# d0-rb/slim-switch-moe-vit

Measured on AMD Instinct MI355X. Metric: images/sec (fwd) ViT-B/16 E=8 @224^2, higher is better.
Workload: dtype f16; 1 GPU; ViT-B/16 Switch-MoE E=8 top-1, 224^2, batch 256/GPU, full eval forward (12 blocks: attention + MoE MLP), fp16 autocast; global_batch=256, compute_streams=1, parallelism=single

## Files before the change

slim-switch-moe-vit_amd/csrc/gemm.hip:

```cpp
#include "smoe_common.h"
#include <type_traits>
#include <cstdlib>

namespace {

typedef __bf16 bf16x8_t __attribute__((ext_vector_type(8)));

constexpr int BM = 128, BN = 128, BK_BYTES = 128;
constexpr int GEMM_THREADS = 256;
constexpr int STAGE_BYTES = (BM + BN) * BK_BYTES;
constexpr int C_PAD = 16;

__device__ __forceinline__ float gelu_erf(float v) {
  const float a = fabsf(v);
  const float z = a * 0.70710678118654752440f;
  const float t = __builtin_amdgcn_rcpf(fmaf(0.3275911f, z, 1.0f));
  float p = fmaf(t, 1.061405429f, -1.453152027f);
  p = fmaf(p, t, 1.421413741f);
  p = fmaf(p, t, -0.284496736f);
  p = fmaf(p, t, 0.254829592f);
  p *= t;
  const float ex = __builtin_amdgcn_exp2f(z * z * -1.4426950408889634f);
  const float erf_abs = fmaf(-p, ex, 1.0f);
  return 0.5f * fmaf(a, erf_abs, v);
// ... 1062 lines not shown
  hipLaunchKernelGGL(kern, dim3(grid), dim3(512), smem, s, (const AB*)PT, (const AB*)QT, (const float*)nullptr, offsets_pad,
                     (const int32_t*)nullptr, E, Lp, R2, (int)SMOE_EPI_NONE, (const int64_t*)nullptr, (const float*)nullptr,
                     (const float*)nullptr, out, tn, tm, R1, (const int64_t*)nullptr, 1);
  SMOE_CHECK_LAUNCH("smoe_grouped_wgrad");
  return 0;
}

template <typename AB>
int launch_wgrad_rows(const void* P, const void* Q, const int32_t* offsets, const int32_t* group_end, int E, int R1, int R2,
                      const void* zero16, float* out, hipStream_t s) {
  constexpr int TBN = 256;
  const int tn = (R2 + TBN - 1) / TBN, tm4 = (R1 + 255) / 256, tm5 = (R1 + 319) / 320;
  const int64_t cus = smoe_num_cus();
  const double c4 = (double)(((int64_t)E * tm4 * tn + cus - 1) / cus), c5 = 1.25 * (double)(((int64_t)E * tm5 * tn + cus - 1) / cus);
  if (c5 < c4) {
    const size_t smem = 2 * (size_t)(320 + TBN) * BK_BYTES;
    auto kern = grouped_gemm_pp256<AB, float, 0, 2, 5>;
    SMOE_ENSURE_SMEM(grouped_gemm_pp256<AB, float, 0, 2, 5>);
    hipLaunchKernelGGL(kern, dim3(E * tm5 * tn), dim3(512), smem, s, (const AB*)P, (const AB*)Q, (const float*)nullptr, offsets,
                       group_end, E, 0, R2, (int)SMOE_EPI_NONE, (const int64_t*)nullptr, (const float*)nullptr,
                       (const float*)zero16, out, tn, tm5, R1, (const int64_t*)nullptr, 1);
  } else {
    const size_t smem = 2 * (size_t)(256 + TBN) * BK_BYTES;
    auto kern = grouped_gemm_pp256<AB, float, 0, 2>;
    SMOE_ENSURE_SMEM(grouped_gemm_pp256<AB, float, 0, 2>);
    hipLaunchKernelGGL(kern, dim3(E * tm4 * tn), dim3(512), smem, s, (const AB*)P, (const AB*)Q, (const float*)nullptr, offsets,
                       group_end, E, 0, R2, (int)SMOE_EPI_NONE, (const int64_t*)nullptr, (const float*)nullptr,
                       (const float*)zero16, out, tn, tm4, R1, (const int64_t*)nullptr, 1);
  }
  SMOE_CHECK_LAUNCH("smoe_grouped_wgrad_rows");
  return 0;
}

template <typename AB, typename OT>
int launch_variant(int variant, const void* A, const void* W, const float* bias, const int32_t* offsets,
                   const int32_t* group_expert, int E, int64_t m_rows_max, int K, int N, int epilogue,
                   const int64_t* row_map, const float* row_scale, const void* residual, void* out, hipStream_t s,
                   const int64_t* a_gather, int a_div, const int32_t* group_end, int64_t out_rows) {
  if constexpr (sizeof(AB) == 2) {
    switch (variant) {
      case 1: return launch_glds<AB, OT, 128, 128, 2, 2, 2>(A, W, bias, offsets, group_expert, E, m_rows_max, K, N, epilogue, row_map, row_scale, residual, out, 8, s);
      case 2: return launch_glds<AB, OT, 256, 128, 2, 2, 1>(A, W, bias, offsets, group_expert, E, m_rows_max, K, N, epilogue, row_map, row_scale, residual, out, 4, s);
      case 3: return launch_glds<AB, OT, 256, 256, 2, 4, 2>(A, W, bias, offsets, group_expert, E, m_rows_max, K, N, epilogue, row_map, row_scale, residual, out, 4, s);
      case 4: {
        const int ntn = (N + 255) / 256;
        const int64_t t256 = ((m_rows_max + 255) / 256 + E / 2) * ntn, t320 = ((m_rows_max + 319) / 320 + E / 2) * ntn;
        const int cus = smoe_num_cus();
        const double c256 = (double)((t256 + cus - 1) / cus) * 1.0, c320 = (double)((t320 + cus - 1) / cus) * 1.25;
        const bool deep = K >= 2048;
        if (c320 <= c256) {
          if (deep) return launch_pp256<AB, OT, 16, 5>(A, W, bias, offsets, group_expert, E, m_rows_max, K, N, epilogue, row_map, row_scale, residual, out, 4, s, a_gather, a_div);
          return launch_pp256<AB, OT, 0, 5>(A, W, bias, offsets, group_expert, E, m_rows_max, K, N, epilogue, row_map, row_scale, residual, out, 4, s, a_gather, a_div);
        }
        if (deep) return launch_pp256<AB, OT, 16, 4>(A, W, bias, offsets, group_expert, E, m_rows_max, K, N, epilogue, row_map, row_scale, residual, out, 4, s, a_gather, a_div);
        return launch_pp256<AB, OT>(A, W, bias, offsets, group_expert, E, m_rows_max, K, N, epilogue, row_map, row_scale, residual, out, 4, s, a_gather, a_div);
      }
#ifdef SMOE_DIAG
      case 5: {
        const char* gm = getenv("SMOE_GROUP_M");
        return launch_pp256<AB, OT, 0, 5>(A, W, bias, offsets, group_expert, E, m_rows_max, K, N, epilogue, row_map, row_scale, residual, out, gm ? atoi(gm) : 4, s, a_gather, a_div);
      }
#else
      case 5: return launch_pp256<AB, OT, 0, 5>(A, W, bias, offsets, group_expert, E, m_rows_max, K, N, epilogue, row_map, row_scale, residual, out, 4, s, a_gather, a_div);
#endif
      case 9: {
        const int ntn = (N + 255) / 256;
        const int64_t t256 = ((m_rows_max + 255) / 256 + E / 2) * ntn, t320 = ((m_rows_max + 319) / 320 + E / 2) * ntn;
        const int cus = smoe_num_cus();
        const double c256 = (double)((t256 + cus - 1) / cus) * 1.0, c320 = (double)((t320 + cus - 1) / cus) * 1.25;
        const bool deep = K >= 2048;
        if (c320 <= c256) {
          if (deep) return launch_ps<AB, OT, 5, true>(A, W, bias, offsets, group_expert, E, m_rows_max, K, N, epilogue, row_map, row_scale, residual, out, 4, s, a_gather, a_div, group_end, out_rows);
          return launch_ps<AB, OT, 5, false>(A, W, bias, offsets, group_expert, E, m_rows_max, K, N, epilogue, row_map, row_scale, residual, out, 4, s, a_gather, a_div, group_end, out_rows);
        }
        if (deep) return launch_ps<AB, OT, 4, true>(A, W, bias, offsets, group_expert, E, m_rows_max, K, N, epilogue, row_map, row_scale, residual, out, 4, s, a_gather, a_div, group_end, out_rows);
        return launch_ps<AB, OT, 4, false>(A, W, bias, offsets, group_expert, E, m_rows_max, K, N, epilogue, row_map, row_scale, residual, out, 4, s, a_gather, a_div, group_end, out_rows);
      }
      case 14: {
        const int ntn = (N + 255) / 256;
        const int64_t t256 = ((m_rows_max + 255) / 256 + E / 2) * ntn, t320 = ((m_rows_max + 319) / 320 + E / 2) * ntn;
        const int cus = smoe_num_cus();
        const double c256 = (double)((t256 + cus - 1) / cus) * 1.0, c320 = (double)((t320 + cus - 1) / cus) * 1.25;
        const bool deep = K >= 2048;
        if (c320 <= c256) {
          if (deep) return launch_ps<AB, OT, 5, true>(A, W, bias, offsets, group_expert, E, m_rows_max, K, N, epilogue, row_map, row_scale, residual, out, 4, s, a_gather, a_div, group_end, out_rows, false);
          return launch_ps<AB, OT, 5, false>(A, W, bias, offsets, group_expert, E, m_rows_max, K, N, epilogue, row_map, row_scale, residual, out, 4, s, a_gather, a_div, group_end, out_rows, false);
        }
        if (deep) return launch_ps<AB, OT, 4, true>(A, W, bias, offsets, group_expert, E, m_rows_max, K, N, epilogue, row_map, row_scale, residual, out, 4, s, a_gather, a_div, group_end, out_rows, false);
        return launch_ps<AB, OT, 4, false>(A, W, bias, offsets, group_expert, E, m_rows_max, K, N, epilogue, row_map, row_scale, residual, out, 4, s, a_gather, a_div, group_end, out_rows, false);
      }
      case 10: return launch_ps<AB, OT, 5, false>(A, W, bias, offsets, group_expert, E, m_rows_max, K, N, epilogue, row_map, row_scale, residual, out, 4, s, a_gather, a_div, group_end, out_rows);
      case 11: return launch_ps<AB, OT, 4, false>(A, W, bias, offsets, group_expert, E, m_rows_max, K, N, epilogue, row_map, row_scale, residual, out, 4, s, a_gather, a_div, group_end, out_rows);
      case 12: return launch_ps<AB, OT, 4, true>(A, W, bias, offsets, group_expert, E, m_rows_max, K, N, epilogue, row_map, row_scale, residual, out, 4, s, a_gather, a_div, group_end, out_rows);
      case 13: return launch_ps<AB, OT, 5, true>(A, W, bias, offsets, group_expert, E, m_rows_max, K, N, epilogue, row_map, row_scale, residual, out, 4, s, a_gather, a_div, group_end, out_rows);
      case 6: return launch_pp256<AB, OT>(A, W, bias, offsets, group_expert, E, m_rows_max, K, N, epilogue, row_map, row_scale, residual, out, 4, s, a_gather, a_div);
      case 7: return launch_pp256<AB, OT, 16, 4>(A, W, bias, offsets, group_expert, E, m_rows_max, K, N, epilogue, row_map, row_scale, residual, out, 4, s, a_gather, a_div);
      case 8: return launch_pp256<AB, OT, 16, 5>(A, W, bias, offsets, group_expert, E, m_rows_max, K, N, epilogue, row_map, row_scale, residual, out, 4, s, a_gather, a_div);
#ifdef SMOE_DIAG
      case 41: return launch_pp256<AB, OT, 1>(A, W, bias, offsets, group_expert, E, m_rows_max, K, N, epilogue, row_map, row_scale, residual, out, 4, s);
      case 42: return launch_pp256<AB, OT, 2>(A, W, bias, offsets, group_expert, E, m_rows_max, K, N, epilogue, row_map, row_scale, residual, out, 4, s);
      case 43: return launch_pp256<AB, OT, 3>(A, W, bias, offsets, group_expert, E, m_rows_max, K, N, epilogue, row_map, row_scale, residual, out, 4, s);
      case 44: return launch_pp256<AB, OT, 4>(A, W, bias, offsets, group_expert, E, m_rows_max, K, N, epilogue, row_map, row_scale, residual, out, 4, s);
      case 46: return launch_pp256<AB, OT, 6>(A, W, bias, offsets, group_expert, E, m_rows_max, K, N, epilogue, row_map, row_scale, residual, out, 4, s);
      case 48: return launch_pp256<AB, OT, 8>(A, W, bias, offsets, group_expert, E, m_rows_max, K, N, epilogue, row_map, row_scale, residual, out, 4, s);
      case 47: return launch_pp256<AB, OT, 7>(A, W, bias, offsets, group_expert, E, m_rows_max, K, N, epilogue, row_map, row_scale, residual, out, 4, s);
#endif
      default: break;
    }
  }
  return launch_t128<AB, OT>(A, W, bias, offsets, group_expert, E, m_rows_max, K, N, epilogue, row_map, row_scale, residual, out, s);
}

template <typename AB>
int dispatch_out(int variant, const void* A, const void* W, const float* bias, const int32_t* offsets, const int32_t* group_expert,
                 int E, int64_t m_rows_max, int K, int N, int epilogue, const int64_t* row_map, const float* row_scale,
                 const void* residual, void* out, int out_dtype, hipStream_t s, const int64_t* a_gather, int a_div,
                 const int32_t* group_end, int64_t out_rows) {
  switch (out_dtype) {
    case SMOE_F32: return launch_variant<AB, float>(variant, A, W, bias, offsets, group_expert, E, m_rows_max, K, N, epilogue, row_map, row_scale, residual, out, s, a_gather, a_div, group_end, out_rows);
    case SMOE_F16: return launch_variant<AB, f16>(variant, A, W, bias, offsets, group_expert, E, m_rows_max, K, N, epilogue, row_map, row_scale, residual, out, s, a_gather, a_div, group_end, out_rows);
    case SMOE_BF16: return launch_variant<AB, bf16_bits>(variant, A, W, bias, offsets, group_expert, E, m_rows_max, K, N, epilogue, row_map, row_scale, residual, out, s, a_gather, a_div, group_end, out_rows);
  }
  smoe_set_error("smoe_grouped_gemm: bad out_dtype %d", out_dtype);
// ... 20 lines not shown
  const size_t cap = sizeof(unsigned long long) * 1024 * 8;
  return (int)hipMemcpyFromSymbol(host_out, HIP_SYMBOL(smoe_clock_stamps), n * 8 < cap ? n * 8 : cap);
}
extern "C" int smoe_clock_clear_stamps() {
  static unsigned long long z[1024 * 8];
  return (int)hipMemcpyToSymbol(HIP_SYMBOL(smoe_clock_stamps), z, sizeof(z));
}
#endif

extern "C" int smoe_grouped_gemm(const void* A, const void* W, const float* bias, const int32_t* offsets,
                                 const int32_t* group_expert, int G, int n_experts, int64_t m_rows_max, int K, int N,
                                 int ab_dtype, int epilogue, const int64_t* row_map, const float* row_scale,
                                 const void* residual, const int64_t* a_gather, int a_div, void* out, int64_t out_rows,
                                 int out_dtype, int variant, const int32_t* group_end, void* stream) {
  SMOE_REQUIRE(offsets && G >= 1 && G <= 65536, "smoe_grouped_gemm: bad G=%d / offsets", G);
  SMOE_REQUIRE(n_experts >= 1 && (group_expert || n_experts == G), "smoe_grouped_gemm: n_experts=%d != G=%d without a group map", n_experts, G);
  SMOE_REQUIRE(m_rows_max >= 0 && m_rows_max < (1ll << 31), "smoe_grouped_gemm: m_rows_max=%lld out of range",
               (long long)m_rows_max);
  SMOE_REQUIRE(K > 0 && N > 0, "smoe_grouped_gemm: bad K=%d N=%d", K, N);
  SMOE_REQUIRE(out_rows >= 0 && (out_rows == 0 || row_map || out_rows >= m_rows_max),
               "smoe_grouped_gemm: out_rows=%lld is smaller than m_rows_max=%lld", (long long)out_rows, (long long)m_rows_max);
  if (out_rows == 0 && !row_map) out_rows = m_rows_max;
  SMOE_REQUIRE(epilogue == SMOE_EPI_NONE || epilogue == SMOE_EPI_GELU || epilogue == SMOE_EPI_GELU_GRAD,
               "smoe_grouped_gemm: bad epilogue %d", epilogue);
  SMOE_REQUIRE(epilogue != SMOE_EPI_GELU_GRAD || (residual && !row_map),
               "smoe_grouped_gemm: SMOE_EPI_GELU_GRAD needs the pre-activations in `residual` and no row_map");
  SMOE_REQUIRE(smoe_dtype_ok(ab_dtype) && smoe_dtype_ok(out_dtype), "smoe_grouped_gemm: bad dtype");
  const int bke = BK_BYTES / smoe_dtype_size(ab_dtype);
  SMOE_REQUIRE(K % bke == 0, "smoe_grouped_gemm: K=%d must be a multiple of %d for this dtype", K, bke);
  SMOE_REQUIRE(N % 8 == 0, "smoe_grouped_gemm: N=%d must be a multiple of 8", N);
  if (m_rows_max == 0) return 0;
  SMOE_REQUIRE(A && W && out, "smoe_grouped_gemm: null pointer");
  if (K % 64 != 0 || smoe_dtype_size(ab_dtype) != 2) variant = 0;
  SMOE_REQUIRE(!a_gather || (variant >= 4 && variant <= 14 && a_div >= 1),
               "smoe_grouped_gemm: a_gather needs variant 4-14 (16-bit operands, K %% 64 == 0)");
  if (variant >= 9 && variant <= 14) {
    const uint64_t a_bytes = (uint64_t)m_rows_max * (uint64_t)K * 2u, w_bytes = (uint64_t)n_experts * (uint64_t)N * (uint64_t)K * 2u;
    if (a_bytes >= (1ull << 32) || w_bytes >= (1ull << 32) || G > 63) variant = variant == 14 ? 4 : variant - 5;
  }
  SMOE_REQUIRE(!group_end || (variant >= 9 && variant <= 14),
               "smoe_grouped_gemm: group_end (separate row ranges per group) needs the persistent kernel: variant 9-14, 16-bit "
               "operands under 4 GiB, K %% 64 == 0, at most 63 groups");
  hipStream_t s = (hipStream_t)stream;
  switch (ab_dtype) {
    case SMOE_F32: return dispatch_out<float>(variant, A, W, bias, offsets, group_expert, G, m_rows_max, K, N, epilogue, row_map, row_scale, residual, out, out_dtype, s, a_gather, a_div, group_end, out_rows);
    case SMOE_F16: return dispatch_out<f16>(variant, A, W, bias, offsets, group_expert, G, m_rows_max, K, N, epilogue, row_map, row_scale, residual, out, out_dtype, s, a_gather, a_div, group_end, out_rows);
    case SMOE_BF16: return dispatch_out<bf16_bits>(variant, A, W, bias, offsets, group_expert, G, m_rows_max, K, N, epilogue, row_map, row_scale, residual, out, out_dtype, s, a_gather, a_div, group_end, out_rows);
  }
  return 1;
}

#ifdef SMOE_FFN_FUSED
extern "C" size_t smoe_expert_ffn_workspace_bytes(int64_t m_rows_max, int G) {
  return sizeof(int32_t) * (size_t)(FUSED_WS_HDR + (m_rows_max + 319) / 320 + (G > 0 ? G : 0) + 8);
}
extern "C" int smoe_expert_ffn(const void* X, const int64_t* a_gather, int a_div, const void* W1, const float* b1, void* H,
                               const void* W2, const float* b2, const int32_t* offsets, const int32_t* group_expert, int G,
                               int n_experts, int64_t m_rows_max, int d_in, int d_hidden, int d_out, int ab_dtype,
                               const int64_t* row_map, const float* row_scale, const void* residual, void* out, int64_t out_rows,
                               int out_dtype, void* workspace, size_t workspace_bytes, void* stream) {
  SMOE_REQUIRE(offsets && G >= 1 && n_experts >= 1 && (group_expert || n_experts == G), "smoe_expert_ffn: bad groups");
  SMOE_REQUIRE(m_rows_max >= 0 && m_rows_max < (1ll << 31) && d_in > 0 && d_hidden > 0 && d_out > 0, "smoe_expert_ffn: bad sizes");
  SMOE_REQUIRE(a_div >= 1, "smoe_expert_ffn: a_div must be >= 1");
  if (m_rows_max == 0) return 0;
  SMOE_REQUIRE(X && W1 && H && W2 && out && workspace, "smoe_expert_ffn: null pointer");
  SMOE_REQUIRE(workspace_bytes >= smoe_expert_ffn_workspace_bytes(m_rows_max, G), "smoe_expert_ffn: workspace too small");
  if ((ab_dtype != SMOE_F16 && ab_dtype != SMOE_BF16) || out_dtype != SMOE_F32) return -1;
  if (d_in % 64 || d_hidden % 64 || d_out % 8 || G > 63) return -1;
  const uint64_t x_bytes = (uint64_t)m_rows_max * (uint64_t)(d_in > d_hidden ? d_in : d_hidden) * 2u;
  const uint64_t w_bytes = (uint64_t)n_experts * (uint64_t)d_hidden * (uint64_t)(d_in > d_out ? d_in : d_out) * 2u;
  if (x_bytes >= (1ull << 32) || w_bytes >= (1ull << 32)) return -1;
  if (out_rows <= 0 || out_rows * (int64_t)d_out * 4 >= (1ll << 31)) return -1;
  if ((int64_t)d_hidden * 320 * 2 >= (1ll << 31)) return -1;
  const int ntn1 = (d_hidden + 255) / 256, ntn2 = (d_out + 255) / 256;
// ... 66 lines not shown
```

slim-switch-moe-vit_amd/csrc/gemm_persistent.h:

```cpp
#ifndef PS_STORE_AUX
#define PS_STORE_AUX 0
#endif
#ifdef SMOE_DIAG
__device__ unsigned long long smoe_diag_stamps[256 * 12 * 16];
__device__ int smoe_diag_flags;
#define PS_NODMA (diag_nodma)
#define PS_IBAR() do { if (!diag_nobar) PP_BARRIER(); } while (0)
#define PS_STAMP(i)                                                                                              \
  do {                                                                                                           \
    if (wave == 0 && lane == 0 && tile_no < 12 && blockIdx.x < 256)                                              \
      smoe_diag_stamps[(blockIdx.x * 12 + tile_no) * 16 + (i)] = __builtin_amdgcn_s_memtime();                   \
  } while (0)
#else
#define PS_STAMP(i) do {} while (0)
#define PS_NODMA false
#define PS_IBAR() PP_BARRIER()
#endif

#ifdef SMOE_CLOCK
__device__ unsigned long long smoe_clock_stamps[1024 * 8];
#define PS_CLOCK(i)                                                                                             \
  do {                                                                                                          \
    if (wave == 0 && lane == 0 && blockIdx.x < 1024) {                                                          \
      unsigned long long t_sh, t_rt;                                                                            \
// ... 14 lines not shown
constexpr int FUSED_WS_HDR = 32;
constexpr int FUSED_WS_LEFT = 16, FUSED_WS_ERR = 17;
constexpr int FUSED_SPIN_LIMIT = 1 << 22;
struct FusedCtl {
  int32_t* ws;
  int mt_lo, cnt;
  int n1, n2, A, B2, G;
  int ntn1, ntn2, gm;
  int stage, slot, j;
  int nk, nid;
};
__device__ __forceinline__ void fused_advance(FusedCtl& fc) {
  if (fc.stage == 1) {
    const int id = fc.slot + fc.G * fc.j;
    if (id < fc.A) { fc.nk = 1; fc.nid = id; ++fc.j; return; }
    fc.nk = 0;
    return;
  }
  if (fc.stage == 2) {
    if (fc.slot < fc.B2) {
      if (fc.j == 0) { fc.nk = 2; fc.nid = fc.slot; fc.j = 1; return; }
    } else {
      const int id = fc.A + (fc.slot - fc.B2) + (fc.G - fc.B2) * fc.j;
      if (id < fc.n1) { fc.nk = 1; fc.nid = id; ++fc.j; return; }
    }
    fc.stage = 3;
    fc.j = 0;
  }
  const int f = fc.B2 + fc.slot + fc.G * fc.j;
  if (f < fc.n2) { fc.nk = 2; fc.nid = f; ++fc.j; return; }
  fc.nk = 0;
}

template <typename AB, typename OT, int AFR, bool DEEP, bool KEEP, bool DIRECT, bool BUF, int FUSED>
__device__ __forceinline__ void ps_body(
    const AB* __restrict__ A, const AB* __restrict__ W, const float* __restrict__ bias,
    const int32_t* __restrict__ offsets, const int32_t* __restrict__ group_expert, int E, int K, int N, int epilogue,
    const int64_t* __restrict__ row_map, const float* __restrict__ row_scale, const OT* residual, OT* out, int n_tiles_n,
    int group_m, const int64_t* __restrict__ a_gather, int a_div, int gather_len, const int32_t* __restrict__ group_end,
    FusedCtl* fc) {
  static_assert(sizeof(AB) == 2, "16-bit operands");
  static_assert(FUSED == 0 || (!KEEP && ((FUSED == 1 && DIRECT) || (FUSED == 2 && BUF))), "fused roles: 1 = producer (direct 16-bit stores), 2 = consumer");
  static_assert(!DIRECT || (sizeof(OT) == 2 && !KEEP), "the direct epilogue stores 16-bit outputs, one output per tile");
  extern __shared__ __attribute__((aligned(16))) char smem[];
  constexpr int TBM = 64 * AFR, TBN = 256, NT = 512, NW = 8;
  constexpr int STAGE = (TBM + TBN) * BK_BYTES;
  constexpr int ASLOTS = TBM / 8 / NW;
  constexpr int SLOTS = 4;
  constexpr int LDS_TOTAL = 160 * 1024;

  const int tid = threadIdx.x, lane = tid & 63;
  const int wave = __builtin_amdgcn_readfirstlane(tid >> 6);
  const int wr = wave >> 2, wc = wave & 3;
  const int fr = lane & 15, fq = lane >> 4;
  const int nk = K / 64;
#ifdef SMOE_DIAG
  const bool diag_nodma = (__builtin_amdgcn_readfirstlane(smoe_diag_flags) & 1) != 0;
  const bool diag_nobar = (__builtin_amdgcn_readfirstlane(smoe_diag_flags) & 2) != 0;
#endif

  int t_off = 0, t_end = 0, t_tb = 0, t_ge = lane;
  {
    const int li = lane < E ? lane : (group_end ? E - 1 : E);
    t_off = offsets[li];
    t_end = group_end ? group_end[li] : offsets[li < E ? li + 1 : E];
    int cnt = lane < E ? (t_end - t_off + TBM - 1) / TBM : 0;
    int incl = cnt;
#pragma unroll
    for (int sft = 1; sft < 64; sft <<= 1) {
      const int up = __shfl_up(incl, sft, 64);
      if (lane >= sft) incl += up;
    }
    t_tb = incl - cnt;
    if (group_expert && lane < E) t_ge = group_expert[lane];
  }
  const int total_mt = __builtin_amdgcn_readlane(t_tb, 63);
// ... 240 lines not shown
    if (a_gather && wave < TBM / 64) {
      int gr = m0 + wave * 64 + lane;
      if (gr >= m_end) gr = m_end - 1;
      __builtin_amdgcn_global_load_lds((const __attribute__((address_space(1))) void*)(a_gather + gr),
                                       (__attribute__((address_space(3))) void*)(smem + LDS_TOTAL - 2048 - TBM * 4 + wave * 256),
                                       4, 0, 0);
    }
  };
  auto issue_bias = [&](int par) {
    if (bias && wave == 0) {
      int col = n0 + lane * 4;
      if (col > N - 4) col = N - 4;
      PS_DMA(bias + (int64_t)e * N + col, bias_lds + par * 1024);
    }
  };

  if constexpr (FUSED == 0) {
    if (!advance()) return;
  } else {
    locate_fused(fc->nid);
    if constexpr (FUSED == 2) fused_wait(mt_next, fused_poll(mt_next));
  }
  if constexpr (FUSED == 0) PS_CLOCK(0);
  {
    int oz = 0;
    asm volatile("" : "+v"(oz));
    setup(lane + oz);
  }
  issue_bias(0);
  issue_kt0();
  if (nk > 1) {
    issue_kt1();
    if constexpr (DEEP) wait_keep2();
    else if constexpr (AFR == 4) asm volatile("s_waitcnt vmcnt(8)" ::: "memory");
    else asm volatile("s_waitcnt vmcnt(9)" ::: "memory");
  } else {
    asm volatile("s_waitcnt vmcnt(0)" ::: "memory");
  }
  PP_BARRIER();

  int tile_no = 0;
  (void)tile_no;
  int cmt = 0;
  for (;; ++tile_no) {
    PS_STAMP(0);
    const int ce = e, cm0 = m0, cm_end = m_end, cn0 = n0;
    cmt = mt_next;
    if constexpr (FUSED != 0) PS_COUNT(4 + FUSED, 1);
    bool more;
    if constexpr (FUSED == 0) {
      tile += t_step;
      more = advance();
    } else {
      fused_advance(*fc);
      more = fc->nk == FUSED;
      if (more) {
        locate_fused(fc->nid);
        if constexpr (FUSED == 2) polled = fused_poll(mt_next);
      }
    }
    if (more) prefetch_rows();
#pragma unroll
    for (int i = 0; i < 2 * AFR; ++i)
#pragma unroll
      for (int j = 0; j < 4; ++j) acc[i][j] = f32x4{0.f, 0.f, 0.f, 0.f};
    if (wr == 1) PP_BARRIER();
    if constexpr (DEEP) {
      for (int t = 0; t < nk; ++t) {
        const int cur = t & 1, nxt = cur ^ 1;
        const bool n1 = (t + 1 < nk), n2 = (t + 2 < nk);
        read_b(cur, 0);
        __builtin_amdgcn_sched_barrier(0);
        read_a(cur, 0);
        if (n1) dma_ah(t + 1, nxt, 1);
        PS_IBAR();
        PS_MFMA(0, 0);
        PS_IBAR();
        read_b(cur, 1);
        if (n1) dma_wh(t + 1, nxt, 0);
        PS_IBAR();
        PS_MFMA(0, 1);
        PS_IBAR();
        read_a(cur, 1);
        if (n2) dma_ah(t + 2, cur, 0);
        PS_IBAR();
        PS_MFMA(1, 1);
        PS_IBAR();
        read_b(cur, 0);
        if (n2) dma_wh(t + 2, cur, 1);
        if (wr == 1) {
          if (n2) wait_keep2();
          else asm volatile("s_waitcnt vmcnt(0)" ::: "memory");
        }
        PS_IBAR();
        PS_MFMA(1, 0);
        if (wr == 0) {
          if (n2) wait_keep2();
          else asm volatile("s_waitcnt vmcnt(0)" ::: "memory");
        }
        PS_IBAR();
      }
    } else {
      for (int t = 0; t < nk; ++t) {
        const int cur = t & 1, nxt = cur ^ 1;
        const bool pre1 = (t >= 1) && (t + 1 < nk);
        const bool pre2 = (t + 2 < nk);
        read_b(cur, 0);
        __builtin_amdgcn_sched_barrier(0);
        read_a(cur, 0);
        if (pre1) dma_a(t + 1, nxt, 2);
        PS_IBAR();
        PS_MFMA(0, 0);
        PS_IBAR();
        read_b(cur, 1);
        if (pre1) dma_w(t + 1, nxt, 0);
        PS_IBAR();
        PS_MFMA(0, 1);
        PS_IBAR();
        read_a(cur, 1);
        if (pre1) dma_w(t + 1, nxt, 2);
        PS_IBAR();
        PS_MFMA(1, 1);
        PS_IBAR();
        read_b(cur, 0);
        if (pre2) dma_a(t + 2, cur, 0);
        if (wr == 1) {
          if (pre2) asm volatile("s_waitcnt vmcnt(2)" ::: "memory");
          else asm volatile("s_waitcnt vmcnt(0)" ::: "memory");
        }
        PS_IBAR();
        PS_MFMA(1, 0);
        if (wr == 0) {
          if (pre2) asm volatile("s_waitcnt vmcnt(2)" ::: "memory");
          else asm volatile("s_waitcnt vmcnt(0)" ::: "memory");
        }
        PS_IBAR();
      }
    }
    if (wr == 0) PP_BARRIER();
    PS_STAMP(1);
    if constexpr (FUSED != 0) {
      if (mt_done >= 0) fused_signal(mt_done);
    }

    PS_STAMP(2);
    int oz = 0;
    asm volatile("" : "+v"(oz));
    const int tid_e = tid + oz, lane_e = tid_e & 63;
    if (more) {
      if constexpr (FUSED == 2) fused_wait(mt_next, polled);
      rows_in_lds = a_gather != nullptr;
      setup(lane_e);
      issue_bias(bias_par ^ 1);
      PS_STAMP(3);
      issue_kt0();
      if constexpr (DIRECT && DEEP) issue_kt1();
    }
    PS_STAMP(4);

    if constexpr (DIRECT) {
      (void)ce;
      const int fr = lane_e & 15, fq = lane_e >> 4;
      f32x4 bv[4];
#pragma unroll
      for (int ni = 0; ni < 4; ++ni) {
        const int nl = wc * 64 + ni * 16 + fq * 4;
        bv[ni] = f32x4{0.f, 0.f, 0.f, 0.f};
        if (bias) bv[ni] = *reinterpret_cast<const f32x4*>(bias_lds + bias_par * 1024 + nl * 4);
      }
      bias_par ^= 1;
      const int rows_here = (cm_end - cm0 < TBM) ? (cm_end - cm0) : TBM;
      const __amdgpu_buffer_rsrc_t rs = __builtin_amdgcn_make_buffer_rsrc(
          reinterpret_cast<char*>(out) + (int64_t)cm0 * N * 2, 0, rows_here * N * 2, 0x00020000);
      const int cq = wc * 64 + (fq & 1) * 16 + (fq >> 1) * 8;
      const uint32_t OOR = 0x80000000u;
      uint32_t off0 = (uint32_t)(((wr * (TBM / 2) + fr) * N + cn0 + cq) * 2);
      const bool ok0 = cn0 + cq < N, ok1 = cn0 + cq + 32 < N;
      const uint32_t row16 = (uint32_t)(16 * N * 2);
#pragma unroll
      for (int mi = 0; mi < 2 * AFR; ++mi) {
#pragma unroll
        for (int q = 0; q < 2; ++q) {
          f32x4 va = acc[mi][2 * q] + bv[2 * q], vb = acc[mi][2 * q + 1] + bv[2 * q + 1];
          if (epilogue == SMOE_EPI_GELU) { va = gelu_fast4(va); vb = gelu_fast4(vb); }
          uint32_t a0, a1, b0, b1;
          pack4<OT>(va, a0, a1);
          pack4<OT>(vb, b0, b1);
          const auto s0 = __builtin_amdgcn_permlane16_swap(a0, b0, false, false);
          const auto s1 = __builtin_amdgcn_permlane16_swap(a1, b1, false, false);
          const u32x4 v = u32x4{s0[0], s1[0], s0[1], s1[1]};
          const uint32_t off = off0 + (uint32_t)(q * 64);
#ifdef FUSED_EXP_PLAIN_STORES
          __builtin_amdgcn_raw_buffer_store_b128(v, rs, (int)((q ? ok1 : ok0) ? off : OOR), 0, PS_STORE_AUX);
#else
          __builtin_amdgcn_raw_buffer_store_b128(v, rs, (int)((q ? ok1 : ok0) ? off : OOR), 0, FUSED == 1 ? 16 : PS_STORE_AUX);
#endif
        }
        off0 += row16;
      }
      PS_STAMP(5);
      if (!more) break;
      if constexpr (DEEP) {
        if constexpr (AFR == 5) asm volatile("s_waitcnt vmcnt(20)" ::: "memory");
        else asm volatile("s_waitcnt vmcnt(16)" ::: "memory");
      } else {
        issue_kt1();
        if (nk > 1) {
          if constexpr (AFR == 5) asm volatile("s_waitcnt vmcnt(29)" ::: "memory");
          else asm volatile("s_waitcnt vmcnt(24)" ::: "memory");
        } else {
          if constexpr (AFR == 5) asm volatile("s_waitcnt vmcnt(20)" ::: "memory");
          else asm volatile("s_waitcnt vmcnt(16)" ::: "memory");
        }
      }
      PP_BARRIER();
      PS_STAMP(12);
      if constexpr (FUSED == 1) mt_done = cmt;
      continue;
    }

    (void)ce;
    const int fr = lane_e & 15, fq = lane_e >> 4;
    const int trow = tid_e / TPR, tcol = tid_e % TPR;
    f32x4 bv[NI];
#pragma unroll
    for (int ni = 0; ni < NI; ++ni) {
      const int nl = wc * TN + ni * 16 + fq * 4;
      bv[ni] = f32x4{0.f, 0.f, 0.f, 0.f};
      if (bias) bv[ni] = *reinterpret_cast<const f32x4*>(bias_lds + bias_par * 1024 + nl * 4);
    }
    bias_par ^= 1;
    const bool use_omap = OMAP && row_map != nullptr;
    if (use_omap && tid_e < TBM) {
      const int m = cm0 + tid_e;
// ... 178 lines not shown
            if (ncol < N) *reinterpret_cast<u32x4*>(reinterpret_cast<char*>(out) + (rbase + ncol) * OB) = v[j];
          }
          if constexpr (KEEP) {
#pragma unroll
            for (int j = 0; j < CPT; ++j) {
              const int ncol = cn0 + (tcol + j * TPR) * (16 / OB);
              const u32x4 h2 = *reinterpret_cast<const u32x4*>(cst2 + r * C_STRIDE + (tcol + j * TPR) * 16);
              if (ncol < N) *reinterpret_cast<u32x4*>(reinterpret_cast<char*>(pre_out) + (rbase + ncol) * OB) = h2;
            }
          }
        }
#pragma unroll
        for (int j = 0; j < CPT; ++j) resv[j] = resn[j];
      }
      if (p == 0) PS_STAMP(7);
      if (p == NPASS - 1) PS_STAMP(11);
      asm volatile("s_waitcnt lgkmcnt(0)" ::: "memory");
      PP_BARRIER();
    }
    PS_STAMP(12);
    if (!more) break;
    issue_kt1();
  }
  if constexpr (FUSED == 0) PS_CLOCK(2);
  if constexpr (FUSED != 0) {
    asm volatile("s_waitcnt vmcnt(0) lgkmcnt(0)" ::: "memory");
    PP_BARRIER();
    if constexpr (FUSED == 1) fused_signal(cmt);
  }
#undef PS_MFMA
#undef PS_DMA
}

template <typename AB, typename OT, int AFR, bool DEEP, bool KEEP = false, bool DIRECT = false, bool BUF = false>
__global__ __launch_bounds__(512, 2) void grouped_gemm_ps(
    const AB* __restrict__ A, const AB* __restrict__ W, const float* __restrict__ bias,
    const int32_t* __restrict__ offsets, const int32_t* __restrict__ group_expert, int E, int K, int N, int epilogue,
    const int64_t* __restrict__ row_map, const float* __restrict__ row_scale, const OT* residual, OT* out, int n_tiles_n,
    int group_m, const int64_t* __restrict__ a_gather, int a_div, int gather_len, const int32_t* __restrict__ group_end) {
  ps_body<AB, OT, AFR, DEEP, KEEP, DIRECT, BUF, 0>(A, W, bias, offsets, group_expert, E, K, N, epilogue, row_map, row_scale, residual,
                                                   out, n_tiles_n, group_m, a_gather, a_div, gather_len, group_end, nullptr);
}

struct FusedPlan { int A, B2; };
__device__ __forceinline__ FusedPlan fused_plan(int cnt, int ntn1, int ntn2, int G, int gm, int c1, int c2) {
  FusedPlan p;
  const int n1 = cnt * ntn1, n2 = cnt * ntn2;
  const int q2 = n2 / G, rem2 = n2 % G;
  p.A = n1;
  p.B2 = 0;
  if (c1 > 0 && rem2 > 0 && rem2 < G) {
    int best_x = -1, best_cost = 0x7fffffff;
    const int x_hi = n1 / G;
    for (int x = x_hi; x >= 0 && x >= x_hi - 8; --x) {
      const int left = n1 - x * G;
      const int y = x + (left + (G - rem2) - 1) / (G - rem2);
      const int heavy = x * c1 + (q2 + 1) * c2, light = y * c1 + q2 * c2;
      const int cost = heavy > light ? heavy : light;
      if (cost < best_cost) { best_cost = cost; best_x = x; }
    }
    const int A = best_x * G;
    const int early_cap = (A / (gm * ntn1)) * gm * ntn2;
    const int B2 = rem2 < early_cap ? rem2 : early_cap;
    if (A < n1 && B2 > 0) { p.A = A; p.B2 = B2; }
  }
  return p;
}

#ifdef SMOE_FFN_FUSED
template <typename AB>
__global__ __launch_bounds__(512, 2) void expert_ffn_fused(
    const AB* __restrict__ X, const int64_t* __restrict__ a_gather, int a_div, int gather_len, const AB* __restrict__ W1,
    const float* __restrict__ b1, AB* H, const AB* __restrict__ W2, const float* __restrict__ b2,
// ... 58 lines not shown
      }
    }
  };
  while (t1 < fc.G) {
    fc.stage = 1;
    fc.slot = t1;
    run_slot();
    if (tid == 0) slot2[0] = __hip_atomic_fetch_add(ws + home, 1, __ATOMIC_RELAXED, __HIP_MEMORY_SCOPE_AGENT);
    __syncthreads();
    t1 = __builtin_amdgcn_readfirstlane(slot2[0]);
    __syncthreads();
  }
  if (t2 < fc.G) {
    const int L = fc.G - fc.B2;
    fc.stage = 2;
    fc.slot = t2 < L ? fc.B2 + t2 : t2 - L;
    run_slot();
  }
  PS_CLOCK(2);
  __syncthreads();
  if (tid == 0) {
    asm volatile("s_waitcnt vmcnt(0)" ::: "memory");
    slot2[0] = __hip_atomic_fetch_add(ws + FUSED_WS_LEFT, 1, __ATOMIC_RELAXED, __HIP_MEMORY_SCOPE_AGENT);
  }
  __syncthreads();
  if (slot2[0] == (int)gridDim.x - 1) {
    for (int i = tid; i < FUSED_WS_HDR + total_mt; i += 512)
      if (i != FUSED_WS_ERR) __hip_atomic_store(ws + i, 0, __ATOMIC_RELAXED, __HIP_MEMORY_SCOPE_AGENT);
  }
}

#endif

template <typename AB, typename OT, int AFR, bool DEEP, bool KEEP = false>
int launch_ps(const void* A, const void* W, const float* bias, const int32_t* offsets, const int32_t* group_expert, int E,
              int64_t m_rows_max, int K, int N, int epilogue, const int64_t* row_map, const float* row_scale,
              const void* residual, void* out, int group_m, hipStream_t s, const int64_t* a_gather, int a_div,
              const int32_t* group_end, int64_t out_rows, bool allow_direct = true) {
  constexpr int TBM = 64 * AFR, TBN = 256;
  const int n_tiles_n = (N + TBN - 1) / TBN;
  const int64_t max_tiles = ((m_rows_max + TBM - 1) / TBM + E) * n_tiles_n;
  int grid = (smoe_num_cus() - smoe_reserved_cus()) & ~7;
  if (grid < 8) grid = 8;
  if (max_tiles < grid) grid = (int)((max_tiles + 7) & ~(int64_t)7);
  int n_block = n_tiles_n <= 4 ? n_tiles_n : 0;
#ifdef SMOE_DIAG
  if (const char* gcap = getenv("SMOE_PS_GRID")) grid = atoi(gcap) & ~7;
  if (const char* ord = getenv("SMOE_PS_NBLOCK")) n_block = atoi(ord);
  if (n_block && n_tiles_n % n_block) n_block = 0;
#endif
  if (n_block) group_m = -(group_m | (n_block << 8));
  if constexpr (!KEEP && sizeof(OT) == 2) {
    if (allow_direct && !row_map && !residual && (epilogue == SMOE_EPI_NONE || epilogue == SMOE_EPI_GELU) && (int64_t)N * TBM * 2 < (1ll << 31)) {
      SMOE_ENSURE_SMEM(grouped_gemm_ps<AB, OT, AFR, DEEP, false, true>);
      hipLaunchKernelGGL((grouped_gemm_ps<AB, OT, AFR, DEEP, false, true>), dim3(grid), dim3(512), 160 * 1024, s, (const AB*)A,
                         (const AB*)W, bias, offsets, group_expert, E, K, N, epilogue, row_map, row_scale, (const OT*)residual,
                         (OT*)out, n_tiles_n, group_m, a_gather, a_div, (int)m_rows_max, group_end);
      SMOE_CHECK_LAUNCH("smoe_grouped_gemm/persistent-direct");
      return 0;
    }
  }
  if constexpr (!KEEP && sizeof(OT) == 4) {
    if (allow_direct && epilogue != SMOE_EPI_GELU_GRAD && out_rows > 0 && out_rows * (int64_t)N * 4 < (1ll << 31)) {
      SMOE_ENSURE_SMEM(grouped_gemm_ps<AB, OT, AFR, DEEP, false, false, true>);
      hipLaunchKernelGGL((grouped_gemm_ps<AB, OT, AFR, DEEP, false, false, true>), dim3(grid), dim3(512), 160 * 1024, s,
                         (const AB*)A, (const AB*)W, bias, offsets, group_expert, E, K, N, epilogue, row_map, row_scale,
                         (const OT*)residual, (OT*)out, n_tiles_n, group_m, a_gather, a_div, (int)m_rows_max, group_end);
      SMOE_CHECK_LAUNCH("smoe_grouped_gemm/persistent-buffer");
      return 0;
    }
  }
  SMOE_ENSURE_SMEM(grouped_gemm_ps<AB, OT, AFR, DEEP, KEEP>);
  hipLaunchKernelGGL((grouped_gemm_ps<AB, OT, AFR, DEEP, KEEP>), dim3(grid), dim3(512), 160 * 1024, s, (const AB*)A, (const AB*)W,
                     bias, offsets, group_expert, E, K, N, epilogue, row_map, row_scale, (const OT*)residual, (OT*)out,
                     n_tiles_n, group_m, a_gather, a_div, (int)m_rows_max, group_end);
  SMOE_CHECK_LAUNCH("smoe_grouped_gemm/persistent");
  return 0;
}
```

Measured before the change: 21610 images/s.

## Add skewed tile-boundary schedule to persistent direct-epilogue grouped GEMM

```diff
diff --git a/slim-switch-moe-vit_amd/csrc/gemm.hip b/slim-switch-moe-vit_amd/csrc/gemm.hip
--- a/slim-switch-moe-vit_amd/csrc/gemm.hip
+++ b/slim-switch-moe-vit_amd/csrc/gemm.hip
@@ -1118,6 +1118,24 @@
   return 0;
 }
 
+template <typename AB, typename OT, int SKEW>
+int launch_ps_auto(const void* A, const void* W, const float* bias, const int32_t* offsets, const int32_t* group_expert, int E,
+                   int64_t m_rows_max, int K, int N, int epilogue, const int64_t* row_map, const float* row_scale,
+                   const void* residual, void* out, hipStream_t s, const int64_t* a_gather, int a_div, const int32_t* group_end,
+                   int64_t out_rows, bool allow_direct) {
+  const int ntn = (N + 255) / 256;
+  const int64_t t256 = ((m_rows_max + 255) / 256 + E / 2) * ntn, t320 = ((m_rows_max + 319) / 320 + E / 2) * ntn;
+  const int cus = smoe_num_cus();
+  const double c256 = (double)((t256 + cus - 1) / cus) * 1.0, c320 = (double)((t320 + cus - 1) / cus) * 1.25;
+  const bool deep = K >= 2048;
+  if (c320 <= c256) {
+    if (deep) return launch_ps<AB, OT, 5, true, false, SKEW>(A, W, bias, offsets, group_expert, E, m_rows_max, K, N, epilogue, row_map, row_scale, residual, out, 4, s, a_gather, a_div, group_end, out_rows, allow_direct);
+    return launch_ps<AB, OT, 5, false, false, SKEW>(A, W, bias, offsets, group_expert, E, m_rows_max, K, N, epilogue, row_map, row_scale, residual, out, 4, s, a_gather, a_div, group_end, out_rows, allow_direct);
+  }
+  if (deep) return launch_ps<AB, OT, 4, true, false, SKEW>(A, W, bias, offsets, group_expert, E, m_rows_max, K, N, epilogue, row_map, row_scale, residual, out, 4, s, a_gather, a_div, group_end, out_rows, allow_direct);
+  return launch_ps<AB, OT, 4, false, false, SKEW>(A, W, bias, offsets, group_expert, E, m_rows_max, K, N, epilogue, row_map, row_scale, residual, out, 4, s, a_gather, a_div, group_end, out_rows, allow_direct);
+}
+
 template <typename AB, typename OT>
 int launch_variant(int variant, const void* A, const void* W, const float* bias, const int32_t* offsets,
                    const int32_t* group_expert, int E, int64_t m_rows_max, int K, int N, int epilogue,
@@ -1149,32 +1167,10 @@
 #else
       case 5: return launch_pp256<AB, OT, 0, 5>(A, W, bias, offsets, group_expert, E, m_rows_max, K, N, epilogue, row_map, row_scale, residual, out, 4, s, a_gather, a_div);
 #endif
-      case 9: {
-        const int ntn = (N + 255) / 256;
-        const int64_t t256 = ((m_rows_max + 255) / 256 + E / 2) * ntn, t320 = ((m_rows_max + 319) / 320 + E / 2) * ntn;
-        const int cus = smoe_num_cus();
-        const double c256 = (double)((t256 + cus - 1) / cus) * 1.0, c320 = (double)((t320 + cus - 1) / cus) * 1.25;
-        const bool deep = K >= 2048;
-        if (c320 <= c256) {
-          if (deep) return launch_ps<AB, OT, 5, true>(A, W, bias, offsets, group_expert, E, m_rows_max, K, N, epilogue, row_map, row_scale, residual, out, 4, s, a_gather, a_div, group_end, out_rows);
-          return launch_ps<AB, OT, 5, false>(A, W, bias, offsets, group_expert, E, m_rows_max, K, N, epilogue, row_map, row_scale, residual, out, 4, s, a_gather, a_div, group_end, out_rows);
-        }
-        if (deep) return launch_ps<AB, OT, 4, true>(A, W, bias, offsets, group_expert, E, m_rows_max, K, N, epilogue, row_map, row_scale, residual, out, 4, s, a_gather, a_div, group_end, out_rows);
-        return launch_ps<AB, OT, 4, false>(A, W, bias, offsets, group_expert, E, m_rows_max, K, N, epilogue, row_map, row_scale, residual, out, 4, s, a_gather, a_div, group_end, out_rows);
-      }
-      case 14: {
-        const int ntn = (N + 255) / 256;
-        const int64_t t256 = ((m_rows_max + 255) / 256 + E / 2) * ntn, t320 = ((m_rows_max + 319) / 320 + E / 2) * ntn;
-        const int cus = smoe_num_cus();
-        const double c256 = (double)((t256 + cus - 1) / cus) * 1.0, c320 = (double)((t320 + cus - 1) / cus) * 1.25;
-        const bool deep = K >= 2048;
-        if (c320 <= c256) {
-          if (deep) return launch_ps<AB, OT, 5, true>(A, W, bias, offsets, group_expert, E, m_rows_max, K, N, epilogue, row_map, row_scale, residual, out, 4, s, a_gather, a_div, group_end, out_rows, false);
-          return launch_ps<AB, OT, 5, false>(A, W, bias, offsets, group_expert, E, m_rows_max, K, N, epilogue, row_map, row_scale, residual, out, 4, s, a_gather, a_div, group_end, out_rows, false);
-        }
-        if (deep) return launch_ps<AB, OT, 4, true>(A, W, bias, offsets, group_expert, E, m_rows_max, K, N, epilogue, row_map, row_scale, residual, out, 4, s, a_gather, a_div, group_end, out_rows, false);
-        return launch_ps<AB, OT, 4, false>(A, W, bias, offsets, group_expert, E, m_rows_max, K, N, epilogue, row_map, row_scale, residual, out, 4, s, a_gather, a_div, group_end, out_rows, false);
-      }
+      case 9: return launch_ps_auto<AB, OT, PS_SKEW>(A, W, bias, offsets, group_expert, E, m_rows_max, K, N, epilogue, row_map, row_scale, residual, out, s, a_gather, a_div, group_end, out_rows, true);
+      case 14: return launch_ps_auto<AB, OT, PS_SKEW>(A, W, bias, offsets, group_expert, E, m_rows_max, K, N, epilogue, row_map, row_scale, residual, out, s, a_gather, a_div, group_end, out_rows, false);
+      case 15: return launch_ps_auto<AB, OT, 2>(A, W, bias, offsets, group_expert, E, m_rows_max, K, N, epilogue, row_map, row_scale, residual, out, s, a_gather, a_div, group_end, out_rows, true);
+      case 16: return launch_ps_auto<AB, OT, 0>(A, W, bias, offsets, group_expert, E, m_rows_max, K, N, epilogue, row_map, row_scale, residual, out, s, a_gather, a_div, group_end, out_rows, true);
       case 10: return launch_ps<AB, OT, 5, false>(A, W, bias, offsets, group_expert, E, m_rows_max, K, N, epilogue, row_map, row_scale, residual, out, 4, s, a_gather, a_div, group_end, out_rows);
       case 11: return launch_ps<AB, OT, 4, false>(A, W, bias, offsets, group_expert, E, m_rows_max, K, N, epilogue, row_map, row_scale, residual, out, 4, s, a_gather, a_div, group_end, out_rows);
       case 12: return launch_ps<AB, OT, 4, true>(A, W, bias, offsets, group_expert, E, m_rows_max, K, N, epilogue, row_map, row_scale, residual, out, 4, s, a_gather, a_div, group_end, out_rows);
@@ -1261,14 +1257,14 @@
   if (m_rows_max == 0) return 0;
   SMOE_REQUIRE(A && W && out, "smoe_grouped_gemm: null pointer");
   if (K % 64 != 0 || smoe_dtype_size(ab_dtype) != 2) variant = 0;
-  SMOE_REQUIRE(!a_gather || (variant >= 4 && variant <= 14 && a_div >= 1),
-               "smoe_grouped_gemm: a_gather needs variant 4-14 (16-bit operands, K %% 64 == 0)");
-  if (variant >= 9 && variant <= 14) {
+  SMOE_REQUIRE(!a_gather || (variant >= 4 && variant <= 16 && a_div >= 1),
+               "smoe_grouped_gemm: a_gather needs variant 4-16 (16-bit operands, K %% 64 == 0)");
+  if (variant >= 9 && variant <= 16) {
     const uint64_t a_bytes = (uint64_t)m_rows_max * (uint64_t)K * 2u, w_bytes = (uint64_t)n_experts * (uint64_t)N * (uint64_t)K * 2u;
-    if (a_bytes >= (1ull << 32) || w_bytes >= (1ull << 32) || G > 63) variant = variant == 14 ? 4 : variant - 5;
-  }
-  SMOE_REQUIRE(!group_end || (variant >= 9 && variant <= 14),
-               "smoe_grouped_gemm: group_end (separate row ranges per group) needs the persistent kernel: variant 9-14, 16-bit "
+    if (a_bytes >= (1ull << 32) || w_bytes >= (1ull << 32) || G > 63) variant = variant >= 14 ? 4 : variant - 5;
+  }
+  SMOE_REQUIRE(!group_end || (variant >= 9 && variant <= 16),
+               "smoe_grouped_gemm: group_end (separate row ranges per group) needs the persistent kernel: variant 9-16, 16-bit "
                "operands under 4 GiB, K %% 64 == 0, at most 63 groups");
   hipStream_t s = (hipStream_t)stream;
   switch (ab_dtype) {
diff --git a/slim-switch-moe-vit_amd/csrc/gemm_persistent.h b/slim-switch-moe-vit_amd/csrc/gemm_persistent.h
--- a/slim-switch-moe-vit_amd/csrc/gemm_persistent.h
+++ b/slim-switch-moe-vit_amd/csrc/gemm_persistent.h
@@ -70,7 +70,7 @@
   fc.nk = 0;
 }
 
-template <typename AB, typename OT, int AFR, bool DEEP, bool KEEP, bool DIRECT, bool BUF, int FUSED>
+template <typename AB, typename OT, int AFR, bool DEEP, bool KEEP, bool DIRECT, bool BUF, int FUSED, bool SKEW = false>
 __device__ __forceinline__ void ps_body(
     const AB* __restrict__ A, const AB* __restrict__ W, const float* __restrict__ bias,
     const int32_t* __restrict__ offsets, const int32_t* __restrict__ group_expert, int E, int K, int N, int epilogue,
@@ -80,6 +80,7 @@
   static_assert(sizeof(AB) == 2, "16-bit operands");
   static_assert(FUSED == 0 || (!KEEP && ((FUSED == 1 && DIRECT) || (FUSED == 2 && BUF))), "fused roles: 1 = producer (direct 16-bit stores), 2 = consumer");
   static_assert(!DIRECT || (sizeof(OT) == 2 && !KEEP), "the direct epilogue stores 16-bit outputs, one output per tile");
+  static_assert(!SKEW || (DIRECT && !DEEP && FUSED == 0), "the skewed boundary is built for the plain-schedule direct epilogue");
   extern __shared__ __attribute__((aligned(16))) char smem[];
   constexpr int TBM = 64 * AFR, TBN = 256, NT = 512, NW = 8;
   constexpr int STAGE = (TBM + TBN) * BK_BYTES;
@@ -386,6 +387,7 @@
   if (nk > 1) {
     issue_kt1();
     if constexpr (DEEP) wait_keep2();
+    else if constexpr (SKEW) asm volatile("s_waitcnt vmcnt(0)" ::: "memory");
     else if constexpr (AFR == 4) asm volatile("s_waitcnt vmcnt(8)" ::: "memory");
     else asm volatile("s_waitcnt vmcnt(9)" ::: "memory");
   } else {
@@ -418,6 +420,35 @@
     for (int i = 0; i < 2 * AFR; ++i)
 #pragma unroll
       for (int j = 0; j < 4; ++j) acc[i][j] = f32x4{0.f, 0.f, 0.f, 0.f};
+    if constexpr (SKEW) {
+      auto solo_kt = [&](int cur) {
+        read_b(cur, 0);
+        __builtin_amdgcn_sched_barrier(0);
+        read_a(cur, 0);
+        PS_MFMA(0, 0);
+        __builtin_amdgcn_sched_barrier(0);
+        read_b(cur, 1);
+        PS_MFMA(0, 1);
+        __builtin_amdgcn_sched_barrier(0);
+        read_a(cur, 1);
+        PS_MFMA(1, 1);
+        __builtin_amdgcn_sched_barrier(0);
+        read_b(cur, 0);
+        PS_MFMA(1, 0);
+        __builtin_amdgcn_sched_barrier(0);
+      };
+      solo_kt(0);
+      if (nk > 1 && wr == 0) solo_kt(1);
+      PP_BARRIER();
+      PS_STAMP(13);
+      if (nk > 2) { dma_a(2, 0, 0); dma_a(2, 0, 2); dma_w(2, 0, 0); dma_w(2, 0, 2); }
+      if (nk > 3) dma_a(3, 1, 0);
+      if (nk > 1 && wr == 1) solo_kt(1);
+      if (nk > 3) asm volatile("s_waitcnt vmcnt(2)" ::: "memory");
+      else asm volatile("s_waitcnt vmcnt(0)" ::: "memory");
+      PP_BARRIER();
+      PS_STAMP(14);
+    }
     if (wr == 1) PP_BARRIER();
     if constexpr (DEEP) {
       for (int t = 0; t < nk; ++t) {
@@ -455,7 +486,7 @@
         PS_IBAR();
       }
     } else {
-      for (int t = 0; t < nk; ++t) {
+      for (int t = SKEW ? 2 : 0; t < nk; ++t) {
         const int cur = t & 1, nxt = cur ^ 1;
         const bool pre1 = (t >= 1) && (t + 1 < nk);
         const bool pre2 = (t + 2 < nk);
@@ -508,7 +539,7 @@
       issue_bias(bias_par ^ 1);
       PS_STAMP(3);
       issue_kt0();
-      if constexpr (DIRECT && DEEP) issue_kt1();
+      if constexpr (DIRECT && (DEEP || SKEW)) issue_kt1();
     }
     PS_STAMP(4);
 
@@ -531,6 +562,12 @@
       uint32_t off0 = (uint32_t)(((wr * (TBM / 2) + fr) * N + cn0 + cq) * 2);
       const bool ok0 = cn0 + cq < N, ok1 = cn0 + cq + 32 < N;
       const uint32_t row16 = (uint32_t)(16 * N * 2);
+      if constexpr (SKEW) {
+        if (more && wr == 1) {
+          asm volatile("s_waitcnt vmcnt(0)" ::: "memory");
+          PP_BARRIER();
+        }
+      }
 #pragma unroll
       for (int mi = 0; mi < 2 * AFR; ++mi) {
 #pragma unroll
@@ -554,6 +591,15 @@
       }
       PS_STAMP(5);
       if (!more) break;
+      if constexpr (SKEW) {
+        if (wr == 0) {
+          if constexpr (AFR == 5) asm volatile("s_waitcnt vmcnt(20)" ::: "memory");
+          else asm volatile("s_waitcnt vmcnt(16)" ::: "memory");
+          PP_BARRIER();
+        }
+        PS_STAMP(12);
+        continue;
+      }
       if constexpr (DEEP) {
         if constexpr (AFR == 5) asm volatile("s_waitcnt vmcnt(20)" ::: "memory");
         else asm volatile("s_waitcnt vmcnt(16)" ::: "memory");
@@ -798,13 +844,13 @@
 #undef PS_DMA
 }
 
-template <typename AB, typename OT, int AFR, bool DEEP, bool KEEP = false, bool DIRECT = false, bool BUF = false>
+template <typename AB, typename OT, int AFR, bool DEEP, bool KEEP = false, bool DIRECT = false, bool BUF = false, bool SKEW = false>
 __global__ __launch_bounds__(512, 2) void grouped_gemm_ps(
     const AB* __restrict__ A, const AB* __restrict__ W, const float* __restrict__ bias,
     const int32_t* __restrict__ offsets, const int32_t* __restrict__ group_expert, int E, int K, int N, int epilogue,
     const int64_t* __restrict__ row_map, const float* __restrict__ row_scale, const OT* residual, OT* out, int n_tiles_n,
     int group_m, const int64_t* __restrict__ a_gather, int a_div, int gather_len, const int32_t* __restrict__ group_end) {
-  ps_body<AB, OT, AFR, DEEP, KEEP, DIRECT, BUF, 0>(A, W, bias, offsets, group_expert, E, K, N, epilogue, row_map, row_scale, residual,
+  ps_body<AB, OT, AFR, DEEP, KEEP, DIRECT, BUF, 0, SKEW>(A, W, bias, offsets, group_expert, E, K, N, epilogue, row_map, row_scale, residual,
                                                    out, n_tiles_n, group_m, a_gather, a_div, gather_len, group_end, nullptr);
 }
 
@@ -929,7 +975,10 @@
 
 #endif
 
-template <typename AB, typename OT, int AFR, bool DEEP, bool KEEP = false>
+#ifndef PS_SKEW
+#define PS_SKEW 1
+#endif
+template <typename AB, typename OT, int AFR, bool DEEP, bool KEEP = false, int SKEW = PS_SKEW>
 int launch_ps(const void* A, const void* W, const float* bias, const int32_t* offsets, const int32_t* group_expert, int E,
               int64_t m_rows_max, int K, int N, int epilogue, const int64_t* row_map, const float* row_scale,
               const void* residual, void* out, int group_m, hipStream_t s, const int64_t* a_gather, int a_div,
@@ -949,6 +998,15 @@
   if (n_block) group_m = -(group_m | (n_block << 8));
   if constexpr (!KEEP && sizeof(OT) == 2) {
     if (allow_direct && !row_map && !residual && (epilogue == SMOE_EPI_NONE || epilogue == SMOE_EPI_GELU) && (int64_t)N * TBM * 2 < (1ll << 31)) {
+      constexpr bool SK = SKEW != 0 && !DEEP;
+      if (SK && (SKEW == 2 || epilogue != SMOE_EPI_GELU)) {
+        SMOE_ENSURE_SMEM(grouped_gemm_ps<AB, OT, AFR, DEEP, false, true, false, SK>);
+        hipLaunchKernelGGL((grouped_gemm_ps<AB, OT, AFR, DEEP, false, true, false, SK>), dim3(grid), dim3(512), 160 * 1024, s,
+                           (const AB*)A, (const AB*)W, bias, offsets, group_expert, E, K, N, epilogue, row_map, row_scale,
+                           (const OT*)residual, (OT*)out, n_tiles_n, group_m, a_gather, a_div, (int)m_rows_max, group_end);
+        SMOE_CHECK_LAUNCH("smoe_grouped_gemm/persistent-direct-skewed");
+        return 0;
+      }
       SMOE_ENSURE_SMEM(grouped_gemm_ps<AB, OT, AFR, DEEP, false, true>);
       hipLaunchKernelGGL((grouped_gemm_ps<AB, OT, AFR, DEEP, false, true>), dim3(grid), dim3(512), 160 * 1024, s, (const AB*)A,
                          (const AB*)W, bias, offsets, group_expert, E, K, N, epilogue, row_map, row_scale, (const OT*)residual,
```

Result: no change. 21650 images/s (median of 6 runs) (+0.2%).
